# neozenith/sqlite-muninn

Hardware: AMD Instinct MI355X
Metric: kNN queries/sec (10k-query batch, k=10, ef=128, 1M x 768 f32 HNSW index) + recall@10 (higher is better)
Workload: dtype f32

## Files before the change

### sqlite-muninn_amd/csrc/mn_device.hpp

```cpp
#pragma once
#include <hip/hip_runtime.h>
#include <stdint.h>

#define MN_WAVE 64

typedef unsigned short mn_lo_t;
struct __align__(16) MnLoMeta {
    float scale;
    float resid;
    float xn_lo;
    float xn_hi;
};
#define MN_LO_MIN_LD 192
__host__ __device__ inline bool mn_lo_enabled(int ld) { return ld >= MN_LO_MIN_LD && (ld & 63) == 0; }
constexpr int MN_ORDER_SSE_V = 0;
constexpr int MN_ORDER_WAVE_V = 1;

struct MnDevIndex {
    const float *vectors;
    const float *norms;
    int *links0;
    int *links_up;
    const int *up_off;
    const signed char *levels;
    const unsigned char *deleted;
    unsigned char *dirty;
    const long long *ids;
    int dim, ld, metric, order;
    int W0, WU;
    int M0, MU;
    int WX;
    int n_slots;
    int n_pool_rows;
    int has_deleted;
    const mn_lo_t *vec_lo;
    const MnLoMeta *lo_meta;
};

#define MN_QC 6
struct MnSearchArgs {
    const float *queries;
    const int *query_slots;
    long long nq;
    int k;
    int ef;
    int entry_slot, max_level;
    long long *out_ids;
    float *out_dists;
    int *out_counts;
    int *sel;
    int *nsel;
    int nlev;
    const int *up_bm_index;
    unsigned *bitmap0;
    long long bm0_words;
    unsigned *bitmap_up;
    long long bmu_words;
    uint2 *cand_ovf;
    int cand_gcap;
    uint2 *res_ovf;
    int res_gcap;
    unsigned long long *counters;
    unsigned long long *q_counters;
    int use_tile;
    int lds_bitmap;
    int *readlog;
    int readcap;
    int *nread;
    int lat_tile_rows;
    unsigned lat_tile_off;
    int surv_lanes;
    int no_spec_rows;
};
size_t mn_lds_optin_limit();
bool mn_lds_grant(const void *kernel, size_t bytes);

#ifndef MN_CAND_LDS
#define MN_CAND_LDS 256
#endif
#ifndef MN_RES_LDS
#define MN_RES_LDS 256
#endif

void mn_module_touch_kernels();
void mn_module_touch_seq();
void mn_module_touch_spec();
void mn_module_touch_build();
void mn_launch_prep_rows(const MnDevIndex &ix, int first_slot, int n, float *norms_out, mn_lo_t *lo_out, MnLoMeta *meta_out,
                         hipStream_t st);
int mn_launch_dist_batch(int metric, int order, const float *d_query, const float *d_rows, long long n, int dim, int ld,
                         float *d_out, hipStream_t st);
size_t mn_dist_batch_lds_bytes(int ld);
size_t mn_search_lds_bytes(int ld, bool tile);
size_t mn_coop_lds_bytes(int ld, bool tile);
size_t mn_spec_commit_min_lds_bytes(int ld);
size_t mn_link_reverse_lds_bytes(int ld, int WX, int nq);
size_t mn_bruteforce_lds_bytes(int ld);
inline size_t mn_row_lds_bytes(int ld) { return (size_t)ld * sizeof(float); }
int mn_launch_search(const MnDevIndex &ix, const MnSearchArgs &a, bool build, hipStream_t st);
void mn_launch_bruteforce(const MnDevIndex &ix, const float *d_queries, long long nq, int k, long long *d_out_ids,
                          float *d_scratch, hipStream_t st);

size_t mn_brute_mfma_scratch_bytes(const MnDevIndex &ix, long long nq, int k, int *n_chunks_out, int *rows_per_chunk_out);
int mn_launch_bruteforce_mfma(const MnDevIndex &ix, const float *d_queries, long long nq, int k, long long *d_out_ids,
                              void *scratch, hipStream_t st);

int mn_index_search_overflow(struct mn_index *x, long long *n_overflow);
void mn_launch_merge_topk(const long long *g_ids, const float *g_dists, const int *g_counts, int world, long long nq, int k,
                          long long *out_ids, float *out_dists, int *out_counts, hipStream_t st);

struct MnLinkArgs {
    int level, M_max;
    int nq, nlev;
    const int *query_slots;
    const int *sel;
    const int *nsel;
    int *t_target;
    int *t_src;
    int *counters;
    int *count;
    int *fill;
    int *binoff;
    int *touched;
    int *bins;
    int *newrows;
    int world, rank;
    int *rec_count;
    int *records;
    int *cls_count;
};
void mn_launch_link(const MnDevIndex &ix, const MnLinkArgs &a, int max_tuples, hipStream_t st);
void mn_launch_link_first(const MnDevIndex &ix, const MnLinkArgs &a, int max_tuples, hipStream_t st);
void mn_launch_link_commit_records(const MnDevIndex &ix, const MnLinkArgs &a, int max_tuples, const int *all_records, int seg,
                                   hipStream_t st);

#define MN_LDS_LIMIT (64 * 1024)
size_t mn_insert_seq_lds_bytes(const MnDevIndex &ix);
void mn_launch_insert_seq(const MnDevIndex &ix, const int *d_slots, int n, int ef, int *d_state, unsigned *bitmap0,
                          long long bm0_words, unsigned *bitmap_up, long long bmu_words, uint2 *cand_ovf, int cand_gcap,
                          uint2 *res_ovf, int res_gcap, unsigned long long *counters, hipStream_t st, int *chlog = nullptr,
                          int chcap = 0);
#define MN_CHLOG_CAP 1024
#define MN_CHLOG_INTS 5

#define MN_RLOG_INTS 5
#define MN_SPEC_SAVE_CAP 8192
void mn_launch_spec_commit(const MnDevIndex &ix, const int *d_slots, int W, int nlev, const int *sel, const int *nsel,
                           const int *readlog, int readcap, const int *nread, int *stamp0, int *stampU, int *sidx0, int *sidxU,
                           int *saved_rows, int *pre_act, int *pre_cnt, int *pre_row, int *why, int epoch, int *d_ncommit,
                           hipStream_t st);

void mn_launch_edge_rows(const MnDevIndex &ix, const int *d_row_slot, const int *d_row_level, int n_rows, int *d_out_nbr,
                         float *d_out_dist, hipStream_t st);
```

### sqlite-muninn_amd/csrc/mn_dist.hpp

```cpp
#pragma once
#include "mn_device.hpp"

#define DEVI __device__ __forceinline__

DEVI int rfl(int v) { return __builtin_amdgcn_readfirstlane(v); }
DEVI unsigned rflu(unsigned v) { return (unsigned)__builtin_amdgcn_readfirstlane((int)v); }
DEVI float u2f(unsigned u) { return __uint_as_float(u); }
DEVI unsigned f2u(float f) { return __float_as_uint(f); }
DEVI double rfl_f64(double v) {
    const unsigned long long b = (unsigned long long)__double_as_longlong(v);
    return __longlong_as_double((long long)(((unsigned long long)rflu((unsigned)(b >> 32)) << 32) | rflu((unsigned)b)));
}


DEVI float cosine_finish(float dot, float na, float nb) {
    float denom = __fmul_rn(sqrtf(na), sqrtf(nb));
    if (denom < 1e-30f)
        return 1.0f;
    return __fsub_rn(1.0f, __fdiv_rn(dot, denom));
}

DEVI float wave_butterfly(float acc) {
#pragma unroll
    for (int m = 32; m >= 1; m >>= 1)
// ... 482 lines not shown
        for (; c + 4 <= steps; c += 4) {
            const float4 b = *reinterpret_cast<const float4 *>(tp + c);
            const float4 a = *reinterpret_cast<const float4 *>(qp + c);
            if (L2) {
                const float d0 = __fsub_rn(a.x, b.x), d1 = __fsub_rn(a.y, b.y), d2 = __fsub_rn(a.z, b.z), d3 = __fsub_rn(a.w, b.w);
                s = __fadd_rn(s, __fmul_rn(d0, d0));
                s = __fadd_rn(s, __fmul_rn(d1, d1));
                s = __fadd_rn(s, __fmul_rn(d2, d2));
                s = __fadd_rn(s, __fmul_rn(d3, d3));
            } else {
                s = __fadd_rn(s, __fmul_rn(a.x, b.x));
                s = __fadd_rn(s, __fmul_rn(a.y, b.y));
                s = __fadd_rn(s, __fmul_rn(a.z, b.z));
                s = __fadd_rn(s, __fmul_rn(a.w, b.w));
            }
        }
        for (; c < steps; c++) {
            const float b = tp[c], a = qp[c];
            float p;
            if (L2) {
                const float d = __fsub_rn(a, b);
                p = __fmul_rn(d, d);
            } else {
                p = __fmul_rn(a, b);
            }
            s = __fadd_rn(s, p);
        }
        const int gb = lane & ~3;
        const float s0 = __shfl(s, gb), s1 = __shfl(s, gb + 1), s2 = __shfl(s, gb + 2), s3 = __shfl(s, gb + 3);
        float sum = __fadd_rn(__fadd_rn(__fadd_rn(s0, s1), s2), s3);
        for (int i = steps * 4; i < ix.dim; i++) {
            const float a = qT[(i & 3) * P + steps], b = tile[gr * RS + (i & 3) * P + steps];
            float p;
            if (L2) {
                const float d = __fsub_rn(a, b);
                p = __fmul_rn(d, d);
            } else {
                p = __fmul_rn(a, b);
            }
            sum = __fadd_rn(sum, p);
        }
        const float got = __shfl(sum, ((lane - t) & 15) << 2);
        if (lane >= t && lane < t + nr)
            mine = got;
    }
    return mine;
}

template <int ORDER, int NCH, bool L2, bool LAT = false>
DEVI float rows_accumulate(const MnDevIndex &ix, const float *q_lds, int myslot, int n, int lane, float *tile = nullptr,
                           int tile_rows = 0) {
    float mine = 0.0f;
    if (ORDER == MN_ORDER_SSE_V) {
        if (LAT && tile) {
            if (tile_rows >= 4)
                return sse_rows_lat_tiled<L2, 4>(ix, q_lds, tile, myslot, n, lane);
            if (tile_rows >= 2)
                return sse_rows_lat_tiled<L2, 2>(ix, q_lds, tile, myslot, n, lane);
        }
#ifdef MN_SSE_TILE_PATH
        if (tile)
            return sse_rows_tiled<L2>(ix, q_lds, tile, myslot, n, lane);
#endif
        for (int t = 0; t < n; t += 16) {
            int r = t + (lane >> 2);
            int s = __shfl(myslot, r < n ? r : n - 1);
            float v = sse_row<L2, LAT, (NCH == 1)>(ix.vectors + (size_t)s * ix.ld, q_lds, ix.dim, lane);
            float got = __shfl(v, ((lane - t) & 15) << 2);
            if (lane >= t && lane < t + 16)
                mine = got;
        }
        return mine;
    }
    if (NCH == 0) {
        for (int t = 0; t < n; t++) {
            int s = __builtin_amdgcn_readlane(myslot, t);
            float v = wave_row_generic<L2>(ix.vectors + (size_t)s * ix.ld, q_lds, ix.ld, lane);
            if (lane == t)
                mine = v;
        }
        return mine;
    }
    constexpr int NC = NCH > 0 ? NCH : 1;
    constexpr int R = (NC <= 3) ? 8 : ((NC <= 6) ? 4 : 2);
    for (int t = 0; t < n; t += R) {
        float4 v[R][NC];
#pragma unroll
        for (int r = 0; r < R; r++) {
            int src = t + r < n ? t + r : n - 1;
            int s = __builtin_amdgcn_readlane(myslot, src);
            const float4 *row = reinterpret_cast<const float4 *>(ix.vectors + (size_t)s * ix.ld);
#pragma unroll
            for (int k = 0; k < NC; k++) {
                int e4 = k * 64 + lane;
                v[r][k] = (e4 * 4 < ix.ld) ? row[e4] : make_float4(0.f, 0.f, 0.f, 0.f);
            }
        }
#pragma unroll
        for (int r = 0; r < R; r++) {
            float acc = 0.0f;
#pragma unroll
            for (int k = 0; k < NC; k++) {
                int e4 = k * 64 + lane;
                if (e4 * 4 < ix.ld) {
                    float4 q = reinterpret_cast<const float4 *>(q_lds)[e4];
                    float4 b = v[r][k];
                    if (L2) {
                        float d0 = __fsub_rn(q.x, b.x), d1 = __fsub_rn(q.y, b.y), d2 = __fsub_rn(q.z, b.z),
                              d3 = __fsub_rn(q.w, b.w);
                        acc = fmaf(d0, d0, acc);
                        acc = fmaf(d1, d1, acc);
                        acc = fmaf(d2, d2, acc);
                        acc = fmaf(d3, d3, acc);
                    } else {
                        acc = fmaf(q.x, b.x, acc);
                        acc = fmaf(q.y, b.y, acc);
                        acc = fmaf(q.z, b.z, acc);
                        acc = fmaf(q.w, b.w, acc);
                    }
                }
            }
            acc = wave_butterfly(acc);
            if (lane == t + r)
                mine = acc;
        }
    }
    return mine;
}

template <int ORDER, int NCH, bool LAT = false>
DEVI float rows_distance(const MnDevIndex &ix, const float *q_lds, float qnorm, int myslot, int n, int lane,
                         float *tile = nullptr, int tile_rows = 0) {
    if (ix.metric == 0) {
        return rows_accumulate<ORDER, NCH, true, LAT>(ix, q_lds, myslot, n, lane, tile, tile_rows);
    }
    float dot = rows_accumulate<ORDER, NCH, false, LAT>(ix, q_lds, myslot, n, lane, tile, tile_rows);
    if (ix.metric == 2)
        return -dot;
    float nb = (lane < n) ? ix.norms[myslot] : 1.0f;
    return cosine_finish(dot, qnorm, nb);
}

DEVI float rows_distance_spread(const MnDevIndex &ix, const float *q_lds, float qnorm, int myslot, int n, int lane, int Q) {
    if (ix.metric == 0)
        return sse_rows_spread<true>(ix, q_lds, myslot, n, lane, Q);
    const float dot = sse_rows_spread<false>(ix, q_lds, myslot, n, lane, Q);
    if (ix.metric == 2)
        return -dot;
    const float nb = (lane < n) ? ix.norms[myslot] : 1.0f;
    return cosine_finish(dot, qnorm, nb);
}


DEVI float lo_deq(unsigned h, float s) { return __fmul_rn((float)__builtin_bit_cast(_Float16, (unsigned short)h), s); }
DEVI double mn_gamma(int n) {
    const double nu = (double)n * 0x1p-24;
    return nu / (1.0 - nu);
}

template <bool L2, int UB>
DEVI void lo_lines(const uint4 *__restrict__ row, const float *q, float s, int lines, int &k, float &acc) {
    for (; k + UB <= lines; k += UB) {
        uint4 v[UB];
#pragma unroll
        for (int u = 0; u < UB; u++)
            v[u] = row[8 * (k + u)];
        __builtin_amdgcn_sched_barrier(0);
#pragma unroll
        for (int u = 0; u < UB; u++) {
            const float4 qa = *reinterpret_cast<const float4 *>(q + 64 * (k + u));
            const float4 qb = *reinterpret_cast<const float4 *>(q + 64 * (k + u) + 4);
            const float qe[8] = {qa.x, qa.y, qa.z, qa.w, qb.x, qb.y, qb.z, qb.w};
            const unsigned w4[4] = {v[u].x, v[u].y, v[u].z, v[u].w};
#pragma unroll
            for (int e = 0; e < 8; e++) {
                const float x = lo_deq((e & 1) ? (w4[e >> 1] >> 16) : (w4[e >> 1] & 0xffffu), s);
                if (L2) {
                    const float d = __fsub_rn(qe[e], x);
                    acc = fmaf(d, d, acc);
                } else {
                    acc = fmaf(qe[e], x, acc);
                }
            }
            __builtin_amdgcn_sched_barrier(0);
        }
    }
}

template <bool L2>
DEVI float lo_rows_accumulate(const MnDevIndex &ix, const float *q_lds, int myslot, float sc, int n, int lane) {
    float mine = 0.0f;
    int ln = lane;
    asm volatile("" : "+v"(ln));
    const int c = ln & 7, r = ln >> 3;
    const int lines = ix.ld >> 6;
    for (int t = 0; t < n; t += 8) {
        const int rr = t + r < n ? t + r : n - 1;
        const int sl = __shfl(myslot, rr);
        const float s = __shfl(sc, rr);
        const uint4 *row = reinterpret_cast<const uint4 *>(ix.vec_lo + (size_t)sl * ix.ld) + c;
        const float *q = q_lds + 8 * c;
        float acc = 0.0f;
        int k = 0;
        lo_lines<L2, 12>(row, q, s, lines, k, acc);
        lo_lines<L2, 4>(row, q, s, lines, k, acc);
        lo_lines<L2, 1>(row, q, s, lines, k, acc);
        acc += quad_xor1(acc);
        acc += quad_xor2(acc);
        acc += __int_as_float(__builtin_amdgcn_ds_swizzle(__float_as_int(acc), 0x101F));
        const float got = __shfl(acc, ((ln - t) & 7) << 3);
        if (ln >= t && ln < t + 8)
            mine = got;
    }
    return mine;
}

struct LoQuery {
    double qs_lo;
    double qn_hi;
};
DEVI LoQuery lo_query(float qsq, int ld) {
    LoQuery lq;
    lq.qs_lo = sqrt((double)qsq) * (1.0 - 0x1p-40);
    const double lost = (double)ld * 0x1p-149;
    lq.qn_hi = sqrt(((double)qsq + lost) / (1.0 - 2.0 * mn_gamma(ld + 8))) * (1.0 + 0x1p-40);
    return lq;
}

DEVI float lo_lower_bound(int metric, float A, const MnLoMeta &m, const LoQuery &lq, int ld) {
    const double a = A, r = m.resid, g = mn_gamma(ld + 8), u = 0x1p-24;
    if (!(fabs(a) <= 3.0e38) || !(r <= 3.0e38))
        return -__builtin_inff();
    double lb;
    if (metric == 0) {
        const double l = (double)sqrtf((float)(fmax(a - (double)ld * 0x1p-147, 0.0) * (1.0 - 4.0 * g))) * (1.0 - 0x1p-21) - 2.0 * r;
        lb = l > 0.0 ? l * l * (1.0 - 4.0 * g) : 0.0;
    } else {
        const double e = 2.0 * (lq.qn_hi * (r + g * (2.0 * (double)m.xn_hi + r)) + (double)ld * 0x1p-147);
        if (metric == 2) {
            lb = -(a + e);
        } else {
            const double den = lq.qs_lo * (double)m.xn_lo * (1.0 - 8.0 * u);
            if (!(den >= 1e-28))
                return -__builtin_inff();
            lb = 1.0 - fmax(a + e, 0.0) / den * (1.0 + 4.0 * u);
        }
    }
    lb -= fabs(lb) * 0x1p-20 + 0x1p-120;
    const float f = __double2float_rd(lb);
    return f == f ? f : -__builtin_inff();
}

template <int ORDER>
DEVI float lds_self_norm(const float *q_lds, int dim, int ld, int lane) {
    if (ORDER == MN_ORDER_SSE_V) {
        float v = sse_row<false>(q_lds, q_lds, dim, lane);
        return __shfl(v, 0);
    }
    return wave_row_generic<false>(q_lds, q_lds, ld, lane);
}

DEVI float lo_rows_bound(const MnDevIndex &ix, const float *q_lds, const LoQuery &lq, int myslot, int n, int lane) {
    MnLoMeta m = {1.0f, __builtin_inff(), 0.0f, 0.0f};
    if (lane < n)
        m = ix.lo_meta[myslot];
    const float A = ix.metric == 0 ? lo_rows_accumulate<true>(ix, q_lds, myslot, m.scale, n, lane)
                                   : lo_rows_accumulate<false>(ix, q_lds, myslot, m.scale, n, lane);
    return lane < n ? lo_lower_bound(ix.metric, A, m, lq, ix.ld) : -__builtin_inff();
}
```

### sqlite-muninn_amd/csrc/mn_index.hip

```cpp
#include "../../include/muninn_hip.h"
#include "mn_guard.hpp"
#include "mn_host.hpp"
#include "mn_device.hpp"
#include "mn_comm.hpp"

#include <algorithm>
#include <cmath>
#include <cstdarg>
#include <cstdio>
#include <cstdlib>
#include <cstring>
#include <string>
#include <unordered_map>
#include <mutex>
#include <vector>

#define MN_MAX_M 512
#define MN_MAX_ROW 2048

static thread_local std::string g_err;

static void set_err(const char *fmt, ...) {
    va_list ap;
    va_start(ap, fmt);
// ... 201 lines not shown
        if (occ >= cap)
            return i;
        live++;
        occ++;
    }
    return -1;
}

struct InsertUndo {
    int first, node_count, max_level, n_pool_rows, old_cap = 0, grew_at = -1;
    unsigned rng;
    int64_t entry_id;
    std::vector<int> old_ht;
};

static void ht_erase_newest(std::vector<int> &t, int cap, const std::vector<int64_t> &ids, int slot) {
    int s = ht_hash(ids[slot], cap);
    for (int i = 0; i < cap; i++) {
        int p = (s + i) & (cap - 1);
        if (t[p] == slot) {
            t[p] = -1;
            return;
        }
    }
}

static void undo_insert(mn_index *x, InsertUndo &u) {
    int hi = x->n_slots;
    if (u.grew_at >= 0) {
        x->ht.swap(u.old_ht);
        x->ht_cap = u.old_cap;
        hi = u.grew_at;
    }
    for (int s = hi - 1; s >= u.first; s--)
        ht_erase_newest(x->ht, x->ht_cap, x->ids, s);
    x->ids.resize((size_t)u.first);
    x->levels.resize((size_t)u.first);
    x->deleted.resize((size_t)u.first);
    x->up_off.resize((size_t)u.first);
    x->n_slots = u.first;
    x->n_pool_rows = u.n_pool_rows;
    x->node_count = u.node_count;
    x->rng_state = u.rng;
    x->entry_id = u.entry_id;
    x->max_level = u.max_level;
    x->meta_uploaded = std::min(x->meta_uploaded, u.first);
    x->staged.clear();
    if (x->host_links_valid) {
        x->h_links0.resize((size_t)x->n_slots * x->W0);
        x->h_links_up.resize((size_t)x->n_pool_rows * x->WU);
    }
}

static int use_device(mn_index *x) {
    if (x->broken) {
        set_err("index unusable: an earlier insert failed after it had begun to rewrite neighbour rows");
        return -1;
    }
    HIPCHK(hipSetDevice(x->device));
    return 0;
}

static MnDevIndex dev_view(mn_index *x) {
    MnDevIndex v;
    v.vectors = x->d_vectors.p;
    v.norms = x->d_norms.p;
    v.links0 = x->d_links0.p;
    v.links_up = x->d_links_up.p;
    v.up_off = x->d_up_off.p;
    v.levels = x->d_levels.p;
    v.deleted = x->d_deleted.p;
    v.dirty = x->d_dirty.p;
    v.ids = x->d_ids.p;
    v.dim = x->dim;
    v.ld = x->ld;
    v.metric = x->metric;
    v.order = x->order;
    v.W0 = x->W0;
    v.WU = x->WU;
    v.M0 = x->M_max0;
    v.MU = x->M;
    v.WX = std::max(x->W0, x->WU);
    v.n_slots = x->n_slots;
    v.n_pool_rows = x->n_pool_rows;
    v.has_deleted = x->n_deleted > 0;
    v.vec_lo = x->d_vec_lo.p;
    v.lo_meta = x->d_lo_meta.p;
    return v;
}

static int host_add_node(mn_index *x, int64_t id, int level, int deleted) {
    int s = x->n_slots;
    x->ids.push_back(id);
    x->levels.push_back((signed char)level);
    x->deleted.push_back((unsigned char)deleted);
    if (level > 0) {
        x->up_off.push_back(x->n_pool_rows);
        x->n_pool_rows += level;
    } else {
        x->up_off.push_back(-1);
    }
    x->n_slots++;
    if (ht_put(x->ht, x->ht_cap, x->ids, s) != 0) {
        x->ids.pop_back();
        x->levels.pop_back();
        x->deleted.pop_back();
        if (level > 0)
            x->n_pool_rows -= level;
        x->up_off.pop_back();
        x->n_slots--;
        return -1;
    }
    if (x->host_links_valid) {
        x->h_links0.resize((size_t)x->n_slots * x->W0, -1);
        x->h_links_up.resize((size_t)x->n_pool_rows * x->WU, -1);
    }
    return s;
}

static int upload_vectors(mn_index *x, int first, const float *vecs, int n, bool src_on_device = false);

static unsigned char *pin_reserve(mn_index *x, size_t need) {
    if (need <= x->pin_cap)
        return x->pin;
    if (hipStreamSynchronize(x->stream) != hipSuccess)
        return nullptr;
    if (x->pin)
        (void)hipHostFree(x->pin);
    x->pin = nullptr;
    x->pin_cap = 0;
    void *p = nullptr;
    if (hipHostMalloc(&p, need * 2, hipHostMallocDefault) != hipSuccess)
        return nullptr;
    x->pin = (unsigned char *)p;
    x->pin_cap = need * 2;
    return x->pin;
}
#define MN_PIN_META 0
#define MN_PIN_IN 64
#define MN_PIN_OUT 96
#define MN_PIN_VEC 256
static size_t pin_log_off(const mn_index *x) { return (MN_PIN_VEC + (size_t)x->ld * sizeof(float) + 63) & ~(size_t)63; }
static size_t pin_insert_bytes(const mn_index *x) {
    return pin_log_off(x) + ((size_t)1 + (size_t)MN_CHLOG_CAP * MN_CHLOG_INTS) * sizeof(int);
}

static int sync_meta(mn_index *x) {
    hipStream_t st = x->stream;
    size_t ns = (size_t)x->n_slots;
    size_t hs = std::max(ns, (size_t)x->slot_hint);
    if (x->d_vectors.reserve(ns * x->ld, true, st, -1, hs * x->ld)) return -1;
    if (x->d_norms.reserve(ns, true, st, -1, hs)) return -1;
    if (mn_lo_enabled(x->ld)) {
        if (x->d_vec_lo.reserve(ns * x->ld, true, st, -1, hs * x->ld)) return -1;
        if (x->d_lo_meta.reserve(ns, true, st, -1, hs)) return -1;
    }
    if (x->d_links0.reserve(ns * x->W0, true, st, 0xFF, hs * x->W0)) return -1;
    if (x->d_links_up.reserve((size_t)std::max(1, x->n_pool_rows) * x->WU, true, st, 0xFF)) return -1;
    if (x->d_up_off.reserve(ns, true, st, -1, hs)) return -1;
    if (x->d_levels.reserve(ns, true, st, -1, hs)) return -1;
    if (x->d_deleted.reserve(ns, true, st, -1, hs)) return -1;
    if (x->d_dirty.reserve(ns, true, st, 0, hs)) return -1;
    if (x->d_ids.reserve(ns, true, st, -1, hs)) return -1;
    int a = x->meta_uploaded, n = x->n_slots - a;
    unsigned char *pin = n == 1 ? pin_reserve(x, pin_insert_bytes(x)) : nullptr;
    if (n == 1 && pin) {
        HIPCHK(hipStreamSynchronize(st));
        int *pi = reinterpret_cast<int *>(pin + MN_PIN_META);
        pi[0] = x->up_off[a];
        reinterpret_cast<unsigned char *>(pi + 1)[0] = (unsigned char)x->levels[a];
        reinterpret_cast<unsigned char *>(pi + 2)[0] = x->deleted[a];
        memcpy(pi + 4, &x->ids[a], sizeof(long long));
        HIPCHK(hipMemcpyAsync(x->d_up_off.p + a, pi, sizeof(int), hipMemcpyHostToDevice, st));
        HIPCHK(hipMemcpyAsync(x->d_levels.p + a, pi + 1, 1, hipMemcpyHostToDevice, st));
        HIPCHK(hipMemcpyAsync(x->d_deleted.p + a, pi + 2, 1, hipMemcpyHostToDevice, st));
        HIPCHK(hipMemcpyAsync(x->d_ids.p + a, pi + 4, sizeof(long long), hipMemcpyHostToDevice, st));
        x->meta_uploaded = x->n_slots;
    } else if (n > 0) {
        HIPCHK(hipMemcpyAsync(x->d_up_off.p + a, x->up_off.data() + a, (size_t)n * sizeof(int), hipMemcpyHostToDevice, st));
        HIPCHK(hipMemcpyAsync(x->d_levels.p + a, x->levels.data() + a, (size_t)n, hipMemcpyHostToDevice, st));
        HIPCHK(hipMemcpyAsync(x->d_deleted.p + a, x->deleted.data() + a, (size_t)n, hipMemcpyHostToDevice, st));
        HIPCHK(hipMemcpyAsync(x->d_ids.p + a, x->ids.data() + a, (size_t)n * sizeof(long long), hipMemcpyHostToDevice, st));
        HIPCHK(hipStreamSynchronize(st));
        x->meta_uploaded = x->n_slots;
    }
    if (!x->load_vecs.empty()) {
        std::vector<float> v;
        v.swap(x->load_vecs);
        const int first = x->load_first;
        x->load_first = -1;
        if (upload_vectors(x, first, v.data(), (int)(v.size() / (size_t)x->dim)))
            return -1;
    }
    return 0;
}

static void prep_rows(mn_index *x, int first, int n) {
    mn_launch_prep_rows(dev_view(x), first, n, x->metric == MN_METRIC_COSINE ? x->d_norms.p : nullptr, x->d_vec_lo.p,
                        x->d_lo_meta.p, x->stream);
}

static int upload_vectors(mn_index *x, int first, const float *vecs, int n, bool src_on_device) {
    hipStream_t st = x->stream;
    const hipMemcpyKind kind = src_on_device ? hipMemcpyDeviceToDevice : hipMemcpyHostToDevice;
    if (n == 1 && !src_on_device && x->pin && x->pin_cap >= pin_insert_bytes(x)) {
        float *pv = reinterpret_cast<float *>(x->pin + MN_PIN_VEC);
        memcpy(pv, vecs, (size_t)x->dim * sizeof(float));
        for (int i = x->dim; i < x->ld; i++)
            pv[i] = 0.0f;
        HIPCHK(hipMemcpyAsync(x->d_vectors.p + (size_t)first * x->ld, pv, (size_t)x->ld * sizeof(float), hipMemcpyHostToDevice, st));
        prep_rows(x, first, 1);
        return 0;
    }
    if (x->ld == x->dim) {
        HIPCHK(hipMemcpyAsync(x->d_vectors.p + (size_t)first * x->ld, vecs, (size_t)n * x->dim * sizeof(float), kind, st));
    } else {
        HIPCHK(hipMemsetAsync(x->d_vectors.p + (size_t)first * x->ld, 0, (size_t)n * x->ld * sizeof(float), st));
        HIPCHK(hipMemcpy2DAsync(x->d_vectors.p + (size_t)first * x->ld, (size_t)x->ld * sizeof(float), vecs,
                                (size_t)x->dim * sizeof(float), (size_t)x->dim * sizeof(float), (size_t)n, kind, st));
    }
    prep_rows(x, first, n);
    HIPCHK(hipStreamSynchronize(st));
    return 0;
}

static size_t d_row_off(const mn_index *x, int slot, int level) {
    return level == 0 ? (size_t)slot * x->W0 : ((size_t)x->up_off[slot] + (level - 1)) * x->WU;
}

static int pull_links(mn_index *x) {
    if (x->host_links_valid)
        return 0;
    x->h_links0.assign((size_t)x->n_slots * x->W0, -1);
    x->h_links_up.assign((size_t)x->n_pool_rows * x->WU, -1);
    const size_t n0 = std::min(x->h_links0.size(), x->d_links0.cap), nu = std::min(x->h_links_up.size(), x->d_links_up.cap);
    if (n0)
        HIPCHK(hipMemcpyAsync(x->h_links0.data(), x->d_links0.p, n0 * sizeof(int), hipMemcpyDeviceToHost, x->stream));
    if (nu)
        HIPCHK(hipMemcpyAsync(x->h_links_up.data(), x->d_links_up.p, nu * sizeof(int), hipMemcpyDeviceToHost, x->stream));
    HIPCHK(hipStreamSynchronize(x->stream));
    x->host_links_valid = true;
    x->dev_links_stale = false;
    x->dev_links_all = false;
    x->h_dirty_rows.clear();
    return 0;
}

static int *h_row(mn_index *x, int slot, int level, int *W);

static int push_links(mn_index *x) {
    if (!x->dev_links_stale)
        return 0;
    if (sync_meta(x))
        return -1;
    if (x->dev_links_all) {
        if (x->n_slots)
            HIPCHK(hipMemcpyAsync(x->d_links0.p, x->h_links0.data(), x->h_links0.size() * sizeof(int), hipMemcpyHostToDevice,
                                  x->stream));
        if (x->n_pool_rows)
            HIPCHK(hipMemcpyAsync(x->d_links_up.p, x->h_links_up.data(), x->h_links_up.size() * sizeof(int),
                                  hipMemcpyHostToDevice, x->stream));
    } else {
        for (const auto &r : x->h_dirty_rows) {
            int W;
            const int *row = h_row(x, r.first, r.second, &W);
            int *dst = (r.second == 0 ? x->d_links0.p : x->d_links_up.p) + d_row_off(x, r.first, r.second);
            HIPCHK(hipMemcpyAsync(dst, row, (size_t)W * sizeof(int), hipMemcpyHostToDevice, x->stream));
        }
    }
    HIPCHK(hipStreamSynchronize(x->stream));
    x->dev_links_stale = false;
    x->dev_links_all = false;
    x->h_dirty_rows.clear();
    return 0;
}

static int *h_row(mn_index *x, int slot, int level, int *W) {
    if (level == 0) {
        *W = x->W0;
        return x->h_links0.data() + (size_t)slot * x->W0;
    }
    *W = x->WU;
    return x->h_links_up.data() + ((size_t)x->up_off[slot] + (level - 1)) * x->WU;
}

static int restride(mn_index *x, bool layer0, int newW) {
    if (pull_links(x))
        return -1;
    std::vector<int> &h = layer0 ? x->h_links0 : x->h_links_up;
    const int oldW = layer0 ? x->W0 : x->WU;
    const size_t rows = layer0 ? (size_t)x->n_slots : (size_t)x->n_pool_rows;
    std::vector<int> nh(rows * (size_t)newW, -1);
    for (size_t r = 0; r < rows; r++)
        memcpy(nh.data() + r * newW, h.data() + r * oldW, (size_t)oldW * sizeof(int));
    h.swap(nh);
    (layer0 ? x->W0 : x->WU) = newW;
    (void)hipStreamSynchronize(x->stream);
    (layer0 ? x->d_links0 : x->d_links_up).release();
    x->dev_links_stale = true;
    x->dev_links_all = true;
    return 0;
}

static int h_row_count(const int *row, int W) {
    int n = 0;
    while (n < W && row[n] >= 0)
        n++;
// ... 1748 lines not shown
```

### sqlite-muninn_amd/csrc/mn_kernels.hip

```cpp
#include "mn_device.hpp"
#include <cstdio>
#include <cstdlib>
#include <mutex>
#include <unordered_map>

#include "mn_dist.hpp"


DEVI double wave_sum_f64(double v) {
#pragma unroll
    for (int m = 32; m >= 1; m >>= 1)
        v += __shfl_xor(v, m);
    return v;
}

template <int ORDER>
__global__ void __launch_bounds__(64)
    k_prep_rows(MnDevIndex ix, int first_slot, int n, float *norms_out, mn_lo_t *lo_out, MnLoMeta *meta_out) {
    extern __shared__ float lds[];
    const int lane = threadIdx.x;
    int slot = first_slot + blockIdx.x;
    if (blockIdx.x >= n)
        return;
    const float *row = ix.vectors + (size_t)slot * ix.ld;
    for (int i = lane; i < ix.ld; i += 64)
        lds[i] = row[i];
    __builtin_amdgcn_s_waitcnt(0);
    __builtin_amdgcn_wave_barrier();
    float nbv = 0.0f;
    if (norms_out) {
        nbv = lds_self_norm<ORDER>(lds, ix.dim, ix.ld, lane);
        if (lane == 0)
            norms_out[slot] = nbv;
    }
    if (!lo_out)
        return;
    float mx = 0.0f;
    bool bad = false;
    for (int i = lane; i < ix.ld; i += 64) {
        const float v = lds[i];
        bad |= !(fabsf(v) <= 3.4028235e38f);
        mx = fmaxf(mx, fabsf(v));
    }
    for (int m = 32; m >= 1; m >>= 1)
        mx = fmaxf(mx, __shfl_xor(mx, m));
    bad = __ballot(bad) != 0;
    int e = 0;
    if (!bad && mx > 0.0f) {
        e = ilogbf(mx) - 14;
        e = e < -140 ? -140 : (e > 127 ? 127 : e);
    }
    const float s = ldexpf(1.0f, e);
    double r2 = 0.0, x2 = 0.0;
    mn_lo_t *lo = lo_out + (size_t)slot * ix.ld;
    for (int i = lane; i < ix.ld; i += 64) {
        const float v = lds[i];
        const _Float16 h = bad ? (_Float16)0.0f : (_Float16)ldexpf(v, -e);
        const unsigned short hb = __builtin_bit_cast(unsigned short, h);
        lo[i] = hb;
        const double dv = (double)v - (double)lo_deq(hb, s);
        r2 += dv * dv;
        x2 += (double)v * (double)v;
    }
    r2 = wave_sum_f64(r2);
    x2 = wave_sum_f64(x2);
    if (lane == 0) {
        MnLoMeta m;
        m.scale = s;
        const double xn = sqrt(x2), rx = sqrt(r2);
        m.xn_lo = norms_out ? __double2float_rd(sqrt((double)nbv) * (1.0 - 0x1p-40)) : __double2float_rd(xn * (1.0 - 0x1p-36));
        m.xn_hi = __double2float_ru(xn * (1.0 + 0x1p-36));
        m.resid = __double2float_ru(rx * (1.0 + 0x1p-36) + 0x1p-140);
        if (bad || !(m.xn_hi <= 3.0e38f) || !(m.resid <= 3.0e38f))
            m.resid = __builtin_inff();
        meta_out[slot] = m;
    }
}

void mn_launch_prep_rows(const MnDevIndex &ix, int first_slot, int n, float *norms_out, mn_lo_t *lo_out, MnLoMeta *meta_out,
                         hipStream_t st) {
    if (n <= 0 || (!norms_out && !lo_out))
        return;
    size_t lds = mn_row_lds_bytes(ix.ld);
    if (ix.order == MN_ORDER_SSE_V)
        hipLaunchKernelGGL(k_prep_rows<MN_ORDER_SSE_V>, dim3(n), dim3(64), lds, st, ix, first_slot, n, norms_out, lo_out, meta_out);
    else
        hipLaunchKernelGGL(k_prep_rows<MN_ORDER_WAVE_V>, dim3(n), dim3(64), lds, st, ix, first_slot, n, norms_out, lo_out, meta_out);
}


template <int ORDER, int NCH>
__global__ void __launch_bounds__(64)
    k_dist_batch(int metric, const float *query, const float *rows, long long n, int dim, int ld, float *out) {
    extern __shared__ float lds[];
    const int lane = threadIdx.x;
    for (int i = lane; i < ld; i += 64)
        lds[i] = i < dim ? query[i] : 0.0f;
    __builtin_amdgcn_s_waitcnt(0);
    __builtin_amdgcn_wave_barrier();
    MnDevIndex ix = {};
    ix.vectors = rows;
    ix.dim = dim;
    ix.ld = ld;
    ix.metric = metric;
    float qnorm = 0.0f;
    if (metric == 1)
        qnorm = lds_self_norm<ORDER>(lds, dim, ld, lane);
    long long base = (long long)blockIdx.x * 64;
    int cnt = (int)((n - base) < 64 ? (n - base) : 64);
    if (cnt <= 0)
        return;
    ix.vectors = rows + (size_t)base * ld;
    int myslot = lane < cnt ? lane : 0;
    float d;
    if (metric == 0) {
        d = rows_accumulate<ORDER, NCH, true>(ix, lds, myslot, cnt, lane);
    } else {
        float dot = rows_accumulate<ORDER, NCH, false>(ix, lds, myslot, cnt, lane);
        if (metric == 2) {
            d = -dot;
        } else {
            float nb = 0.0f;
            for (int t = 0; t < cnt; t++) {
                const float *row = ix.vectors + (size_t)t * ld;
                float *tmp = lds + ld;
                for (int i = lane; i < ld; i += 64)
                    tmp[i] = row[i];
                __builtin_amdgcn_s_waitcnt(0);
                __builtin_amdgcn_wave_barrier();
                float v = lds_self_norm<ORDER>(tmp, dim, ld, lane);
                __builtin_amdgcn_wave_barrier();
                if (lane == t)
                    nb = v;
            }
            d = cosine_finish(dot, qnorm, nb);
        }
    }
    if (lane < cnt)
        out[base + lane] = d;
}

static int pick_nch(int ld) {
    int need = (ld + 255) / 256;
    if (need <= 1) return 1;
    if (need <= 2) return 2;
    if (need <= 3) return 3;
    if (need <= 4) return 4;
    if (need <= 6) return 6;
    if (need <= 8) return 8;
    return 0;
}

size_t mn_dist_batch_lds_bytes(int ld) { return (size_t)ld * sizeof(float) * 2; }

template <int ORDER, int NCH>
static int launch_dist_batch(int metric, const float *d_query, const float *d_rows, long long n, int dim, int ld, float *d_out,
                             hipStream_t st) {
    const size_t lds = mn_dist_batch_lds_bytes(ld);
    if (lds > mn_lds_optin_limit() || !mn_lds_grant(reinterpret_cast<const void *>(k_dist_batch<ORDER, NCH>), lds))
        return -1;
    hipLaunchKernelGGL((k_dist_batch<ORDER, NCH>), dim3((unsigned)((n + 63) / 64)), dim3(64), lds, st, metric, d_query, d_rows, n,
                       dim, ld, d_out);
    return hipGetLastError() == hipSuccess ? 0 : -1;
}

int mn_launch_dist_batch(int metric, int order, const float *d_query, const float *d_rows, long long n, int dim, int ld,
                         float *d_out, hipStream_t st) {
    if (n <= 0)
        return 0;
    if (order == MN_ORDER_SSE_V)
        return launch_dist_batch<MN_ORDER_SSE_V, 0>(metric, d_query, d_rows, n, dim, ld, d_out, st);
#define MN_DB(N) \
    case N:      \
        return launch_dist_batch<MN_ORDER_WAVE_V, N>(metric, d_query, d_rows, n, dim, ld, d_out, st);
    switch (pick_nch(ld)) {
        MN_DB(1) MN_DB(2) MN_DB(3) MN_DB(4) MN_DB(6) MN_DB(8)
    default:
        return launch_dist_batch<MN_ORDER_WAVE_V, 0>(metric, d_query, d_rows, n, dim, ld, d_out, st);
    }
#undef MN_DB
}

#include "mn_beam.hpp"

template <int ORDER, int NCH, bool BUILD, bool WIDE, bool LAT = false, bool LP = false>
DEVI void beam_query(const MnDevIndex &ix, const MnSearchArgs &a, const long long qi, const int lane, unsigned char *smem,
                     CoopCtx *coop, unsigned *lds_bitmap = nullptr) {
    uint2 *cand_l = reinterpret_cast<uint2 *>(smem);
    uint2 *res_l = cand_l + MN_CAND_LDS;
    int *scratch = reinterpret_cast<int *>(res_l + MN_RES_LDS);
    float *q = reinterpret_cast<float *>(scratch + 64);
    float *tile = q + ix.ld;

    int qslot = -1;
    const float *qsrc;
    if (BUILD) {
        qslot = a.query_slots[qi];
        qsrc = ix.vectors + (size_t)qslot * ix.ld;
    } else {
        qsrc = a.queries + (size_t)qi * ix.dim;
    }
    for (int i = lane; i < ix.ld; i += 64)
        q[i] = i < ix.dim ? qsrc[i] : 0.0f;
    __builtin_amdgcn_s_waitcnt(0);
    __builtin_amdgcn_wave_barrier();

    WaveCtx w;
    w.q = q;
    w.tile = (ORDER == MN_ORDER_SSE_V && a.use_tile) ? tile : nullptr;
    w.scratch = scratch;
    w.n_dist = 0;
    w.n_exp = 0;
    w.qnorm = 0.0f;
    if (ix.metric == 1)
        w.qnorm = BUILD ? ix.norms[qslot] : lds_self_norm<ORDER>(q, ix.dim, ix.ld, lane);
    if (coop) {
        w.coop = coop;
        w.no_spec_rows = a.no_spec_rows;
        if (lane == 0)
            *coop->qnorm = w.qnorm;
    }
    if (LP) {
        w.lq = lo_query(ix.metric == 1 ? w.qnorm : lds_self_norm<ORDER>(q, ix.dim, ix.ld, lane), ix.ld);
        w.lp_on = w.lq.qn_hi <= 1.0e300;
        w.lq.qs_lo = rfl_f64(w.lq.qs_lo);
        w.lq.qn_hi = rfl_f64(w.lq.qn_hi);
        w.qnorm = u2f(rflu(f2u(w.qnorm)));
        w.sv_lanes = a.surv_lanes;
    }
    if (BUILD && a.readlog) {
        w.rlog = a.readlog + (size_t)qi * a.readcap * MN_RLOG_INTS;
        w.rcap = a.readcap;
    }

    WHeap cand, res;
    cand.l = cand_l;
    cand.lcap = MN_CAND_LDS;
    cand.g = reinterpret_cast<unsigned long long *>(a.cand_ovf + (size_t)qi * a.cand_gcap);
    cand.gcap = a.cand_gcap;
    cand.size = 0;
    cand.ovf = 0;
    res.l = res_l;
    res.lcap = MN_RES_LDS;
    res.g = reinterpret_cast<unsigned long long *>(a.res_ovf + (size_t)qi * a.res_gcap);
    res.gcap = a.res_gcap;
    res.size = 0;
    res.ovf = 0;

    unsigned *bm0 = lds_bitmap ? lds_bitmap : a.bitmap0 + (size_t)qi * a.bm0_words;
    int cur = a.entry_slot;

    if (!BUILD) {
        for (int l = a.max_level; l > 0; l--)
            cur = greedy_layer<ORDER, NCH, false, WIDE>(ix, w, cur, l, lane);
        if (LAT)
            beam_layer_auto<ORDER, NCH, false, WIDE>(ix, w, cand, res, bm0, a.bm0_words, cur, 0, a.ef, lane);
        else
            beam_layer<ORDER, NCH, false, WIDE, false, LP>(ix, w, cand, res, bm0, cur, 0, a.ef, lane);
        int count = res.size;
        int outn = count < a.k ? count : a.k;
        for (int i = count - 1; i >= 0; i--) {
            uint2 it = res_take(res, i, count, lane);
            if (i < a.k && lane == 0) {
                a.out_ids[qi * a.k + i] = ix.ids[it.y];
                a.out_dists[qi * a.k + i] = -u2f(it.x);
            }
        }
        if (lane == 0) {
            for (int i = outn; i < a.k; i++) {
                a.out_ids[qi * a.k + i] = -1;
                a.out_dists[qi * a.k + i] = 0.0f;
            }
            a.out_counts[qi] = outn;
        }
    } else {
        const int level = ix.levels[qslot];
        for (int l = a.max_level; l > level; l--)
            cur = greedy_layer<ORDER, NCH, false, WIDE, LAT>(ix, w, cur, l, lane);
        int start = level < a.max_level ? level : a.max_level;
        for (int l = start; l >= 0; l--) {
            unsigned *bm = bm0;
            if (l > 0)
                bm = a.bitmap_up + ((size_t)a.up_bm_index[qi] * a.max_level + (l - 1)) * a.bmu_words;
            if (LAT)
                beam_layer_auto<ORDER, NCH, false, WIDE, true>(ix, w, cand, res, bm, l > 0 ? a.bmu_words : a.bm0_words, cur, l, a.ef, lane);
            else
                beam_layer<ORDER, NCH, false, WIDE>(ix, w, cand, res, bm, cur, l, a.ef, lane);
            const int M_max = (l == 0) ? ix.M0 : ix.MU;
            int count = res.size;
            int keep = count < M_max ? count : M_max;
            int *sel = a.sel + ((size_t)qi * a.nlev + l) * ix.M0;
            int first = cur;
            for (int i = count - 1; i >= 0; i--) {
                uint2 it = res_take(res, i, count, lane);
                if (i < keep && lane == 0)
                    sel[i] = (int)it.y;
                if (i == 0)
                    first = (int)it.y;
            }
            if (lane == 0)
                a.nsel[qi * a.nlev + l] = keep;
            if (count > 0)
                cur = first;
        }
    }
    if (lane == 0) {
        if (BUILD && a.readlog)
            a.nread[qi] = LAT ? w.nr : a.readcap + 1;
        if (a.q_counters) {
            a.q_counters[(size_t)qi * MN_QC + 0] = w.n_dist;
            a.q_counters[(size_t)qi * MN_QC + 1] = w.n_exp;
            a.q_counters[(size_t)qi * MN_QC + 2] = (cand.ovf || res.ovf) ? 1ull : 0ull;
            a.q_counters[(size_t)qi * MN_QC + 3] = w.n_skip;
            a.q_counters[(size_t)qi * MN_QC + 4] = w.n_l8;
            a.q_counters[(size_t)qi * MN_QC + 5] = w.n_l16;
        } else {
            atomicAdd(&a.counters[0], w.n_dist);
            atomicAdd(&a.counters[1], w.n_exp);
            if (cand.ovf || res.ovf)
                atomicAdd(&a.counters[2], 1ull);
            if (LP && w.n_skip)
                atomicAdd(&a.counters[3], w.n_skip);
            if (LP && w.n_l8)
                atomicAdd(&a.counters[4], w.n_l8);
            if (LP && w.n_l16)
                atomicAdd(&a.counters[5], w.n_l16);
        }
    }
}

template <int ORDER, int NCH, bool BUILD, bool WIDE = false, bool LP = false>
__global__ void __launch_bounds__(64) k_beam(MnDevIndex ix, MnSearchArgs a) {
    extern __shared__ __align__(16) unsigned char smem[];
    if ((long long)blockIdx.x >= a.nq)
        return;
    beam_query<ORDER, NCH, BUILD, WIDE, false, LP>(ix, a, blockIdx.x, threadIdx.x, smem, nullptr);
}

#define MN_COOP_WAVES 8
template <int ORDER, int NCH, bool BUILD, bool WIDE = false>
__global__ void __launch_bounds__(MN_COOP_WAVES * 64) k_beam_coop(MnDevIndex ix, MnSearchArgs a, size_t base_lds) {
    extern __shared__ __align__(16) unsigned char smem[];
    if ((long long)blockIdx.x >= a.nq)
        return;
    const int lane = threadIdx.x & 63;
    CoopCtx c;
    c.n = reinterpret_cast<int *>(smem + base_lds);
    c.qnorm = reinterpret_cast<float *>(c.n + 1);
    c.list = c.n + 4;
    c.dist = reinterpret_cast<float *>(c.list + 64);
    c.nw = blockDim.x >> 6;
    c.wv = threadIdx.x >> 6;
    if (a.lat_tile_rows > 0) {
        c.tile = reinterpret_cast<float *>(smem + a.lat_tile_off) + (size_t)c.wv * mn_lat_tile_floats(ix.ld, a.lat_tile_rows);
        c.tile_rows = a.lat_tile_rows;
    }
    unsigned *lbm = nullptr;
    if (!BUILD && a.lds_bitmap) {
        lbm = reinterpret_cast<unsigned *>(smem + base_lds) + 4 + 64 + 64;
        for (long long i = threadIdx.x; i < a.bm0_words; i += blockDim.x)
            lbm[i] = 0u;
        __syncthreads();
    }
    if (c.wv == 0) {
        beam_query<ORDER, NCH, BUILD, WIDE, true>(ix, a, blockIdx.x, lane, smem, &c, lbm);
        if (lane == 0)
            *c.n = -1;
        __syncthreads();
    } else {
        const float *q = reinterpret_cast<const float *>(smem + (size_t)(MN_CAND_LDS + MN_RES_LDS) * sizeof(uint2) + 64 * sizeof(int));
        coop_helper<ORDER, NCH>(ix, q, c, lane);
    }
}

size_t mn_search_lds_bytes(int ld, bool tile) {
    size_t b = (size_t)(MN_CAND_LDS + MN_RES_LDS) * sizeof(uint2) + 64 * sizeof(int) + (size_t)ld * sizeof(float);
    if (tile)
        b += MN_TILE_FLOATS * sizeof(float);
    if (const char *pad = getenv("MN_LDS_PAD_BYTES"))
        b += (size_t)atoi(pad);
    return b;
}
size_t mn_coop_lds_bytes(int ld, bool tile) { return ((mn_search_lds_bytes(ld, tile) + 15) & ~(size_t)15) + (4 + 64 + 64) * sizeof(int); }

size_t mn_lds_optin_limit() {
    static std::mutex mu;
    static std::unordered_map<int, size_t> lims;
    int dev = 0;
    (void)hipGetDevice(&dev);
    std::lock_guard<std::mutex> lk(mu);
    auto it = lims.find(dev);
    if (it != lims.end())
        return it->second;
    size_t lim = 64 * 1024;
    const char *e = getenv("MN_LDS_OPTIN");
    int v = 0;
    if (!(e && atoi(e) == 0) && hipDeviceGetAttribute(&v, hipDeviceAttributeSharedMemPerBlockOptin, dev) == hipSuccess && v > 64 * 1024)
        lim = (size_t)v;
    (void)hipGetLastError();
    lims[dev] = lim;
    return lim;
}
bool mn_lds_grant(const void *kern, size_t bytes) {
    if (bytes <= 64 * 1024)
        return true;
    static std::mutex mu;
    struct Seen {
        size_t granted = 0;
        size_t refused = (size_t)-1;
    };
    static std::unordered_map<unsigned long long, Seen> seen;
    int dev = 0;
    (void)hipGetDevice(&dev);
    const unsigned long long key = (unsigned long long)reinterpret_cast<uintptr_t>(kern) * 64ull + (unsigned)(dev & 63);
    std::lock_guard<std::mutex> lk(mu);
    Seen &sn = seen[key];
    if (sn.granted >= bytes)
        return true;
    if (bytes >= sn.refused)
        return false;
    const bool ok = hipFuncSetAttribute(kern, hipFuncAttributeMaxDynamicSharedMemorySize, (int)bytes) == hipSuccess;
    if (ok) {
        sn.granted = bytes;
    } else {
        (void)hipGetLastError();
        sn.refused = bytes;
    }
    return ok;
}
template <typename K> static bool lds_grant(K kern, size_t bytes) { return mn_lds_grant(reinterpret_cast<const void *>(kern), bytes); }

template <int ORDER, int NCH, bool BUILD, bool WIDE>
static void launch_coop(const MnDevIndex &ix, MnSearchArgs a, size_t base, size_t tot, hipStream_t st) {
    const char *te = getenv("MN_LAT_TILE");
    if (ORDER == MN_ORDER_SSE_V && ix.ld >= 256 && !(te && atoi(te) == 0)) {
        const size_t off = (tot + 15) & ~(size_t)15;
        for (int rows = 4; rows >= 2; rows >>= 1) {
            const size_t need = off + (size_t)MN_COOP_WAVES * mn_lat_tile_floats(ix.ld, rows) * sizeof(float);
            if (need <= mn_lds_optin_limit() && lds_grant(k_beam_coop<ORDER, NCH, BUILD, WIDE>, need)) {
                a.lat_tile_rows = rows;
                a.lat_tile_off = (unsigned)off;
                tot = need;
                break;
            }
        }
    }
    if (getenv("MN_LAT_DEBUG"))
        fprintf(stderr, "[mn] k_beam_coop: distance tile of %d rows per wavefront, %zu bytes of LDS\n", a.lat_tile_rows, tot);
    hipLaunchKernelGGL((k_beam_coop<ORDER, NCH, BUILD, WIDE>), dim3((unsigned)a.nq), dim3(MN_COOP_WAVES * 64), tot, st, ix, a, base);
}

template <int ORDER, int NCH>
static void launch_beam(const MnDevIndex &ix, const MnSearchArgs &a, bool build, hipStream_t st) {
    dim3 grid((unsigned)a.nq), block(64);
    size_t lds = mn_search_lds_bytes(ix.ld, ORDER == MN_ORDER_SSE_V && a.use_tile);
    const bool wide = ix.WX > 64;
    const char *co = getenv("MN_COOP");
    if (a.nq <= 128 && !(co && atoi(co) == 0)) {
        const size_t base = (lds + 15) & ~(size_t)15;
        const size_t tot = mn_coop_lds_bytes(ix.ld, ORDER == MN_ORDER_SSE_V && a.use_tile) +
                           (!build && a.lds_bitmap ? (size_t)a.bm0_words * sizeof(unsigned) : 0);
        if (wide) {
            if (build)
                launch_coop<ORDER, NCH, true, true>(ix, a, base, tot, st);
            else
                launch_coop<ORDER, NCH, false, true>(ix, a, base, tot, st);
        } else if (build)
            launch_coop<ORDER, NCH, true, false>(ix, a, base, tot, st);
        else
            launch_coop<ORDER, NCH, false, false>(ix, a, base, tot, st);
        return;
    }
    const char *lp = getenv("MN_LOWPREC_FILTER");
    if (!build && ix.vec_lo && ix.lo_meta && !(lp && atoi(lp) == 0)) {
        MnSearchArgs al = a;
        const char *sv = getenv("MN_SURVIVOR_LANES");
        const int svl = sv ? atoi(sv) : 0;
        al.surv_lanes = (svl == 4 || svl == 8 || svl == 16) ? svl : 0;
        if (wide)
            hipLaunchKernelGGL((k_beam<ORDER, NCH, false, true, true>), grid, block, lds, st, ix, al);
        else
            hipLaunchKernelGGL((k_beam<ORDER, NCH, false, false, true>), grid, block, lds, st, ix, al);
        return;
    }
    if (wide) {
        if (build)
            hipLaunchKernelGGL((k_beam<ORDER, NCH, true, true>), grid, block, lds, st, ix, a);
        else
            hipLaunchKernelGGL((k_beam<ORDER, NCH, false, true>), grid, block, lds, st, ix, a);
    } else if (build)
        hipLaunchKernelGGL((k_beam<ORDER, NCH, true>), grid, block, lds, st, ix, a);
    else
        hipLaunchKernelGGL((k_beam<ORDER, NCH, false>), grid, block, lds, st, ix, a);
}

int mn_launch_search(const MnDevIndex &ix, const MnSearchArgs &a, bool build, hipStream_t st) {
    if (a.nq <= 0)
        return 0;
    if (ix.order == MN_ORDER_SSE_V) {
        const char *qe = getenv("MN_SSE_QUAD");
        if (MN_SSE_QUAD2 > 0 && (ix.dim >> 4) >= MN_SSE_QUAD2 && !(qe && atoi(qe) == 0))
            launch_beam<MN_ORDER_SSE_V, 1>(ix, a, build, st);
        else
            launch_beam<MN_ORDER_SSE_V, 0>(ix, a, build, st);
        return 0;
    }
    switch (pick_nch(ix.ld)) {
    case 1: launch_beam<MN_ORDER_WAVE_V, 1>(ix, a, build, st); break;
    case 2: launch_beam<MN_ORDER_WAVE_V, 2>(ix, a, build, st); break;
    case 3: launch_beam<MN_ORDER_WAVE_V, 3>(ix, a, build, st); break;
    case 4: launch_beam<MN_ORDER_WAVE_V, 4>(ix, a, build, st); break;
    case 6: launch_beam<MN_ORDER_WAVE_V, 6>(ix, a, build, st); break;
    case 8: launch_beam<MN_ORDER_WAVE_V, 8>(ix, a, build, st); break;
    default: launch_beam<MN_ORDER_WAVE_V, 0>(ix, a, build, st); break;
    }
    return 0;
}


template <int ORDER, int NCH>
__global__ void __launch_bounds__(64)
    k_edge_rows(MnDevIndex ix, const int *row_slot, const int *row_level, int n_rows, int *out_nbr, float *out_dist) {
    extern __shared__ __align__(16) unsigned char smem[];
    const int lane = threadIdx.x;
    const int r = blockIdx.x;
    if (r >= n_rows)
        return;
    float *q = reinterpret_cast<float *>(smem);
    const int s = row_slot[r], level = row_level[r];
// ... 108 lines not shown
```

Measured before the change: 516,400.

## Replace fp16 low-precision row copies with packed 10-bit integer codes

The low-precision shadow copy of each index row moves from fp16 with a power-of-two scale to signed 10-bit integer codes with a per-row max/511 scale, packed three per 32-bit word. This cuts the bytes read per candidate distance from 2 to about 1.33 per dimension, easing memory bandwidth during beam search. The query buffer in LDS is padded to 96-float lines, and the lo distance loop is retuned for 12 codes per lane-chunk. The coarser quantization enlarges the residual bound, which may force more exact-distance refinements and could affect recall or the amount of re-checking work.

```diff
diff --git a/sqlite-muninn_amd/csrc/mn_device.hpp b/sqlite-muninn_amd/csrc/mn_device.hpp
--- a/sqlite-muninn_amd/csrc/mn_device.hpp
+++ b/sqlite-muninn_amd/csrc/mn_device.hpp
@@ -4,7 +4,11 @@
 
 #define MN_WAVE 64
 
-typedef unsigned short mn_lo_t;
+typedef unsigned mn_lo_t;
+#define MN_LO_BITS 10
+#define MN_LO_CMAX 511
+#define MN_LO_LINE_CODES 96
+#define MN_LO_LINE_WORDS 32
 struct __align__(16) MnLoMeta {
     float scale;
     float resid;
@@ -13,6 +17,13 @@
 };
 #define MN_LO_MIN_LD 192
 __host__ __device__ inline bool mn_lo_enabled(int ld) { return ld >= MN_LO_MIN_LD && (ld & 63) == 0; }
+__host__ __device__ inline int mn_lo_lines(int ld) { return (ld + MN_LO_LINE_CODES - 1) / MN_LO_LINE_CODES; }
+__host__ __device__ inline size_t mn_lo_row_words(int ld) { return (size_t)mn_lo_lines(ld) * MN_LO_LINE_WORDS; }
+__host__ __device__ inline int mn_lo_q_floats(int ld) { return mn_lo_enabled(ld) ? mn_lo_lines(ld) * MN_LO_LINE_CODES : ld; }
+__host__ __device__ inline int mn_lo_code(unsigned w, int f) { return (int)(w << (32 - MN_LO_BITS * (f + 1))) >> (32 - MN_LO_BITS); }
+__host__ __device__ inline unsigned mn_lo_pack(int c0, int c1, int c2) {
+    return ((unsigned)c0 & 0x3ffu) | (((unsigned)c1 & 0x3ffu) << 10) | (((unsigned)c2 & 0x3ffu) << 20);
+}
 constexpr int MN_ORDER_SSE_V = 0;
 constexpr int MN_ORDER_WAVE_V = 1;
 
diff --git a/sqlite-muninn_amd/csrc/mn_dist.hpp b/sqlite-muninn_amd/csrc/mn_dist.hpp
--- a/sqlite-muninn_amd/csrc/mn_dist.hpp
+++ b/sqlite-muninn_amd/csrc/mn_dist.hpp
@@ -658,7 +658,7 @@
 }
 
 
-DEVI float lo_deq(unsigned h, float s) { return __fmul_rn((float)__builtin_bit_cast(_Float16, (unsigned short)h), s); }
+DEVI float lo_deq(int c, float s) { return __fmul_rn((float)c, s); }
 DEVI double mn_gamma(int n) {
     const double nu = (double)n * 0x1p-24;
     return nu / (1.0 - nu);
@@ -674,13 +674,14 @@
         __builtin_amdgcn_sched_barrier(0);
 #pragma unroll
         for (int u = 0; u < UB; u++) {
-            const float4 qa = *reinterpret_cast<const float4 *>(q + 64 * (k + u));
-            const float4 qb = *reinterpret_cast<const float4 *>(q + 64 * (k + u) + 4);
-            const float qe[8] = {qa.x, qa.y, qa.z, qa.w, qb.x, qb.y, qb.z, qb.w};
+            const float4 qa = *reinterpret_cast<const float4 *>(q + MN_LO_LINE_CODES * (k + u));
+            const float4 qb = *reinterpret_cast<const float4 *>(q + MN_LO_LINE_CODES * (k + u) + 4);
+            const float4 qc = *reinterpret_cast<const float4 *>(q + MN_LO_LINE_CODES * (k + u) + 8);
+            const float qe[12] = {qa.x, qa.y, qa.z, qa.w, qb.x, qb.y, qb.z, qb.w, qc.x, qc.y, qc.z, qc.w};
             const unsigned w4[4] = {v[u].x, v[u].y, v[u].z, v[u].w};
 #pragma unroll
-            for (int e = 0; e < 8; e++) {
-                const float x = lo_deq((e & 1) ? (w4[e >> 1] >> 16) : (w4[e >> 1] & 0xffffu), s);
+            for (int e = 0; e < 12; e++) {
+                const float x = lo_deq(mn_lo_code(w4[e / 3], e % 3), s);
                 if (L2) {
                     const float d = __fsub_rn(qe[e], x);
                     acc = fmaf(d, d, acc);
@@ -699,17 +700,18 @@
     int ln = lane;
     asm volatile("" : "+v"(ln));
     const int c = ln & 7, r = ln >> 3;
-    const int lines = ix.ld >> 6;
+    const int lines = mn_lo_lines(ix.ld);
+    const size_t row_words = mn_lo_row_words(ix.ld);
     for (int t = 0; t < n; t += 8) {
         const int rr = t + r < n ? t + r : n - 1;
         const int sl = __shfl(myslot, rr);
         const float s = __shfl(sc, rr);
-        const uint4 *row = reinterpret_cast<const uint4 *>(ix.vec_lo + (size_t)sl * ix.ld) + c;
-        const float *q = q_lds + 8 * c;
+        const uint4 *row = reinterpret_cast<const uint4 *>(ix.vec_lo + (size_t)sl * row_words) + c;
+        const float *q = q_lds + 12 * c;
         float acc = 0.0f;
         int k = 0;
-        lo_lines<L2, 12>(row, q, s, lines, k, acc);
-        lo_lines<L2, 4>(row, q, s, lines, k, acc);
+        lo_lines<L2, 8>(row, q, s, lines, k, acc);
+        lo_lines<L2, 2>(row, q, s, lines, k, acc);
         lo_lines<L2, 1>(row, q, s, lines, k, acc);
         acc += quad_xor1(acc);
         acc += quad_xor2(acc);
diff --git a/sqlite-muninn_amd/csrc/mn_index.hip b/sqlite-muninn_amd/csrc/mn_index.hip
--- a/sqlite-muninn_amd/csrc/mn_index.hip
+++ b/sqlite-muninn_amd/csrc/mn_index.hip
@@ -377,7 +377,7 @@
     if (x->d_vectors.reserve(ns * x->ld, true, st, -1, hs * x->ld)) return -1;
     if (x->d_norms.reserve(ns, true, st, -1, hs)) return -1;
     if (mn_lo_enabled(x->ld)) {
-        if (x->d_vec_lo.reserve(ns * x->ld, true, st, -1, hs * x->ld)) return -1;
+        if (x->d_vec_lo.reserve(ns * mn_lo_row_words(x->ld), true, st, -1, hs * mn_lo_row_words(x->ld))) return -1;
         if (x->d_lo_meta.reserve(ns, true, st, -1, hs)) return -1;
     }
     if (x->d_links0.reserve(ns * x->W0, true, st, 0xFF, hs * x->W0)) return -1;
diff --git a/sqlite-muninn_amd/csrc/mn_kernels.hip b/sqlite-muninn_amd/csrc/mn_kernels.hip
--- a/sqlite-muninn_amd/csrc/mn_kernels.hip
+++ b/sqlite-muninn_amd/csrc/mn_kernels.hip
@@ -45,22 +45,31 @@
     for (int m = 32; m >= 1; m >>= 1)
         mx = fmaxf(mx, __shfl_xor(mx, m));
     bad = __ballot(bad) != 0;
-    int e = 0;
-    if (!bad && mx > 0.0f) {
-        e = ilogbf(mx) - 14;
-        e = e < -140 ? -140 : (e > 127 ? 127 : e);
-    }
-    const float s = ldexpf(1.0f, e);
+    float s = __fdiv_rn(mx, (float)MN_LO_CMAX);
+    bad |= !(s >= 1.17549435e-38f && s <= 3.4028235e38f);
+    if (bad)
+        s = 0.0f;
     double r2 = 0.0, x2 = 0.0;
-    mn_lo_t *lo = lo_out + (size_t)slot * ix.ld;
-    for (int i = lane; i < ix.ld; i += 64) {
-        const float v = lds[i];
-        const _Float16 h = bad ? (_Float16)0.0f : (_Float16)ldexpf(v, -e);
-        const unsigned short hb = __builtin_bit_cast(unsigned short, h);
-        lo[i] = hb;
-        const double dv = (double)v - (double)lo_deq(hb, s);
-        r2 += dv * dv;
-        x2 += (double)v * (double)v;
+    mn_lo_t *lo = lo_out + (size_t)slot * mn_lo_row_words(ix.ld);
+    const int words = (int)mn_lo_row_words(ix.ld);
+    for (int w = lane; w < words; w += 64) {
+        int c[3];
+#pragma unroll
+        for (int f = 0; f < 3; f++) {
+            const int i = 3 * w + f;
+            c[f] = 0;
+            if (i < ix.ld) {
+                const float v = lds[i];
+                if (!bad) {
+                    const float t = rintf(__fdiv_rn(v, s));
+                    c[f] = (int)fminf(fmaxf(t, -(float)MN_LO_CMAX), (float)MN_LO_CMAX);
+                }
+                const double dv = (double)v - (double)lo_deq(c[f], s);
+                r2 += dv * dv;
+                x2 += (double)v * (double)v;
+            }
+        }
+        lo[w] = mn_lo_pack(c[0], c[1], c[2]);
     }
     r2 = wave_sum_f64(r2);
     x2 = wave_sum_f64(x2);
@@ -190,7 +199,8 @@
     uint2 *res_l = cand_l + MN_CAND_LDS;
     int *scratch = reinterpret_cast<int *>(res_l + MN_RES_LDS);
     float *q = reinterpret_cast<float *>(scratch + 64);
-    float *tile = q + ix.ld;
+    const int qf = mn_lo_q_floats(ix.ld);
+    float *tile = q + qf;
 
     int qslot = -1;
     const float *qsrc;
@@ -200,7 +210,7 @@
     } else {
         qsrc = a.queries + (size_t)qi * ix.dim;
     }
-    for (int i = lane; i < ix.ld; i += 64)
+    for (int i = lane; i < qf; i += 64)
         q[i] = i < ix.dim ? qsrc[i] : 0.0f;
     __builtin_amdgcn_s_waitcnt(0);
     __builtin_amdgcn_wave_barrier();
@@ -374,7 +384,7 @@
 }
 
 size_t mn_search_lds_bytes(int ld, bool tile) {
-    size_t b = (size_t)(MN_CAND_LDS + MN_RES_LDS) * sizeof(uint2) + 64 * sizeof(int) + (size_t)ld * sizeof(float);
+    size_t b = (size_t)(MN_CAND_LDS + MN_RES_LDS) * sizeof(uint2) + 64 * sizeof(int) + (size_t)mn_lo_q_floats(ld) * sizeof(float);
     if (tile)
         b += MN_TILE_FLOATS * sizeof(float);
     if (const char *pad = getenv("MN_LDS_PAD_BYTES"))
```

Measured after the change: 596,000, median of 6. 1.15x the previous value.
